# s-elkazdadi/ddp-pinocchio

Measured on AMD Instinct MI355X. Metric: DDP iterations/sec (fwd+bwd sweep), Talos nq=38 T=200, higher is better.
Workload: dtype f64

## Files before the change

ddp_pinocchio_amd/csrc/bwd.hip:

```cpp
#include <stdio.h>
#include <stdlib.h>

#include "internal.h"

namespace {

struct BwdParams {
  Dims d;
  const int64_t* ne;
  const int64_t* Epre;
  const double *lfx, *lfxx, *lx, *lu, *lxx, *lux, *luu, *fx, *fu, *fxx, *fux, *fuu;
  const double *eq_val, *eq_x, *eq_u, *eq_xx, *eq_ux, *eq_uu;
  const double *x, *mult_val, *mult_jac;
  double *fb_origin, *fb_val, *fb_jac, *vx_trace, *vxx_trace;
  double *ws_V, *ws_Q, *reg, *mu;
  int32_t* status;
  int64_t* restarts;
  const BwdJob* jobs;
  const BwdJob* jobs_half;
  int32_t njobs_half;
  int32_t half_mode;
  int32_t packed;
  const double *u, *ctrl_lo, *ctrl_hi;
  double* box_stat;
  int32_t has_tensors;
  int32_t sym_tensors;
};

constexpr int BS = 256;
typedef double f64x2 __attribute__((ext_vector_type(2)));

__global__ __launch_bounds__(BS) void bwd_init(BwdParams p) {
  const int b = blockIdx.x;
  const int s = p.status[b];
  if (s == 2) return;
  const int64_t n = p.d.n;
  double* Vx = p.ws_V + (int64_t)b * (n + n * n);
  double* Vxx = Vx + n;
  const double* lfx = p.lfx + (int64_t)b * n;
  const double* lfxx = p.lfxx + (int64_t)b * n * n;
  for (int64_t i = threadIdx.x; i < n; i += BS) Vx[i] = lfx[i];
  for (int64_t i = threadIdx.x; i < n * n; i += BS) Vxx[i] = lfxx[i];
  __syncthreads();
  if (threadIdx.x == 0 && s == 1) p.status[b] = 0;
}

template <int OC>
__device__ __forceinline__ void contract_slab(const double* __restrict__ Tn, int O_rt, int L, const double* s_v,
                                              double* s_part, double* out, int out_stride) {
  const int O = OC > 0 ? OC : O_rt;
  const int hp = O >> 1;
  const int ld = hp + 1;
  const int total = hp * L;
  const f64x2* __restrict__ T2 = reinterpret_cast<const f64x2*>(Tn);
  const int tid = threadIdx.x;
#pragma unroll 4
  for (int f = tid; f < total; f += BS) {
    const f64x2 a = __builtin_nontemporal_load(&T2[f]);
    const int j = f / hp;
    const int ip = f - j * hp;
    s_part[j * ld + ip] = s_v[2 * ip] * a.x + s_v[2 * ip + 1] * a.y;
  }
  __syncthreads();
  for (int j = tid; j < L; j += BS) {
    double s = 0.0;
    const double* pj = s_part + j * ld;
    for (int k = 0; k < hp; ++k) s += pj[k];
    out[j * out_stride] += s;
  }
  __syncthreads();
}

template <int NC, int MC>
__global__ __launch_bounds__(BS) void bwd_assemble(BwdParams p, int64_t t) {
  const int b = blockIdx.y;
  if (p.status[b] != 0) return;
  const BwdJob job = p.jobs[blockIdx.x];
  const int n = NC > 0 ? NC : (int)p.d.n;
  const int m = MC > 0 ? MC : (int)p.d.m;
  const int64_t T = p.d.T;
  const int e = (int)p.ne[t];
  const int64_t Eo = p.Epre[t];
  const int64_t Etot = p.d.Etot;
  const double mu = p.mu[b];
  const int tid = threadIdx.x;
  const int kind = job.kind, c0 = job.c0, cn = job.cn;
  const int rows = kind == 0 ? n + m : m;

  const double* Vx = p.ws_V + (int64_t)b * (n + (int64_t)n * n);
  const double* Vxx = Vx + n;
  double* Q = p.ws_Q + (int64_t)b * (n + m + (int64_t)n * n + (int64_t)m * n + (int64_t)m * m);
  double* Qx = Q;
  double* Qu = Qx + n;
  double* Qxx = Qu + m;
  double* Qux = Qxx + (int64_t)n * n;
  double* Quu = Qux + (int64_t)m * n;

  const int64_t bt = (int64_t)b * T + t;
  const double* fx = p.fx + bt * n * n;
  const double* fu = p.fu + bt * n * m;
  const double* eqv = p.eq_val + (int64_t)b * Etot + Eo;
  const double* eqx = p.eq_x + ((int64_t)b * Etot + Eo) * n;
  const double* equ = p.eq_u + ((int64_t)b * Etot + Eo) * m;
  const double* pe = p.mult_val + (int64_t)b * Etot + Eo;
  const double* pex = p.mult_jac + ((int64_t)b * Etot + Eo) * n;
// ... 333 lines not shown
      double s = r[i];
      for (int l = 0; l < i; ++l) s -= A[i + l * lda] * r[l];
      r[i] = s / A[i + i * lda];
    }
    for (int i = m - 1; i >= 0; --i) {
      double s = r[i];
      for (int l = i + 1; l < m; ++l) s -= A[l + i * lda] * r[l];
      r[i] = s / A[i + i * lda];
    }
  }
  __syncthreads();

  double* fbo = p.fb_origin + bt * nx;
  double* fbk = p.fb_val + bt * m;
  double* fbK = p.fb_jac + bt * m * n;
  const double* xt = p.x + ((int64_t)b * (T + 1) + t) * nx;
  for (int i = tid; i < nx; i += BS) fbo[i] = xt[i];
  for (int i = tid; i < m; i += BS) fbk[i] = R[i];
  for (int idx = tid; idx < m * n; idx += BS) fbK[idx] = R[idx % m + (idx / m + 1) * ldr];

  for (int i = tid; i < n; i += BS) {
    double s = 0.0;
    for (int l = 0; l < m; ++l) s += S[l + i * ldr] * R[l];
    const double v = Qx[i] + s;
    Vx[i] = v;
    if (p.vx_trace) p.vx_trace[bt * n + i] = v;
  }
  for (int idx = tid; idx < n * n; idx += BS) {
    const int i = idx % n, j = idx / n;
    double s = 0.0;
    const double* si = S + i * ldr;
    const double* kj = R + (j + 1) * ldr;
    for (int l = 0; l < m; ++l) s += si[l] * kj[l];
    const double v = Qxx[idx] + s;
    Vxx[idx] = v;
    if (p.vxx_trace) p.vxx_trace[bt * n * n + idx] = v;
  }
  if (t == 0 && tid == 0) p.status[b] = 2;
}

#include "bwd_fast.h"
#include "bwd_split.h"
#include "bwd_v2.h"

size_t assemble_lds_bytes(const ddp_hip_ctx* ctx, int cn_max) {
  const Dims& d = ctx->d;
  int64_t L = d.n > d.m ? d.n : d.m;
  int64_t words = d.n + d.emax + d.n * cn_max + (d.n + d.m) * cn_max + (d.n / 2 + 1) * L;
  return (size_t)words * sizeof(double);
}
size_t gains_lds_bytes(const ddp_hip_ctx* ctx) {
  const Dims& d = ctx->d;
  int64_t ld = d.m | 1;
  int64_t words = ld * d.m + ld * (d.n + 1) + ld * d.n;
  if (ctx->flags & DDP_HIP_FLAG_CONTROL_BOUNDS) words += ld * d.m + 9 * d.m;
  return (size_t)words * sizeof(double);
}

BwdParams make_params(ddp_hip_ctx* ctx, const SweepPlan& plan) {
  BwdParams p{};
  p.d = ctx->d;
  p.ne = ctx->ne_d;
  p.Epre = ctx->Epre_d;
  auto S = [&](int s) { return ctx->seq[s].ptr; };
  p.lfx = S(DDP_HIP_SEQ_LFX); p.lfxx = S(DDP_HIP_SEQ_LFXX);
  p.lx = S(DDP_HIP_SEQ_LX); p.lu = S(DDP_HIP_SEQ_LU); p.lxx = S(DDP_HIP_SEQ_LXX); p.lux = S(DDP_HIP_SEQ_LUX); p.luu = S(DDP_HIP_SEQ_LUU);
  p.fx = S(DDP_HIP_SEQ_FX); p.fu = S(DDP_HIP_SEQ_FU);
  p.fxx = S(DDP_HIP_SEQ_FXX); p.fux = S(DDP_HIP_SEQ_FUX); p.fuu = S(DDP_HIP_SEQ_FUU);
  p.eq_val = S(DDP_HIP_SEQ_EQ_VAL); p.eq_x = S(DDP_HIP_SEQ_EQ_X); p.eq_u = S(DDP_HIP_SEQ_EQ_U);
  p.eq_xx = S(DDP_HIP_SEQ_EQ_XX); p.eq_ux = S(DDP_HIP_SEQ_EQ_UX); p.eq_uu = S(DDP_HIP_SEQ_EQ_UU);
  p.x = S(DDP_HIP_SEQ_X);
  p.u = S(DDP_HIP_SEQ_U); p.ctrl_lo = S(DDP_HIP_SEQ_CTRL_LO); p.ctrl_hi = S(DDP_HIP_SEQ_CTRL_HI); p.box_stat = S(DDP_HIP_SEQ_BOX_STAT);
  p.mult_val = S(DDP_HIP_SEQ_MULT_VAL); p.mult_jac = S(DDP_HIP_SEQ_MULT_JAC);
  p.fb_origin = S(DDP_HIP_SEQ_FB_ORIGIN); p.fb_val = S(DDP_HIP_SEQ_FB_VAL); p.fb_jac = S(DDP_HIP_SEQ_FB_JAC);
  p.vx_trace = S(DDP_HIP_SEQ_VX_TRACE); p.vxx_trace = S(DDP_HIP_SEQ_VXX_TRACE);
  p.ws_V = ctx->ws_V; p.ws_Q = ctx->ws_Q; p.reg = ctx->reg_d; p.mu = ctx->mu_d;
  p.status = ctx->status_d; p.restarts = ctx->restarts_d;
  p.sym_tensors = plan.sym ? 1 : 0;
  p.jobs = plan.sym ? ctx->jobs_sym_d : ctx->jobs_d;
  p.jobs_half = plan.half_mode ? ctx->jobs_half_d : nullptr;
  p.njobs_half = plan.half_mode ? ctx->njobs_half : 0;
  p.half_mode = plan.half_mode;
  p.packed = plan.packed ? 1 : 0;
  p.has_tensors = (ctx->flags & DDP_HIP_FLAG_NO_TENSORS) ? 0 : 1;
  return p;
}

template <int NC, int MC, bool BOX = false>
int launch_sweep(ddp_hip_ctx* ctx, const BwdParams& p, size_t lds_a, size_t lds_g) {
  const Dims& d = ctx->d;
  hipLaunchKernelGGL(bwd_init, dim3((unsigned)d.batch), dim3(BS), 0, ctx->stream, p);
  for (int64_t t = d.T - 1; t >= 0; --t) {
    prof_begin(ctx, DDP_HIP_K_BWD_ASSEMBLE);
    hipLaunchKernelGGL((bwd_assemble<NC, MC>), dim3((unsigned)ctx->njobs, (unsigned)d.batch), dim3(BS), lds_a, ctx->stream, p, t);
    prof_end(ctx, DDP_HIP_K_BWD_ASSEMBLE);
    prof_begin(ctx, DDP_HIP_K_BWD_GAINS);
    hipLaunchKernelGGL((bwd_gains<NC, MC, BOX>), dim3((unsigned)d.batch), dim3(BS), lds_g, ctx->stream, p, t);
    prof_end(ctx, DDP_HIP_K_BWD_GAINS);
  }
  HIP_TRY(hipGetLastError());
  return DDP_HIP_OK;
}

template <int NC, int MC, bool BOX>
int enqueue_sweep_v2(ddp_hip_ctx* ctx, const BwdParams& p) {
  const Dims& d = ctx->d;
  const int cn_max = ctx->cbx > ctx->cbu ? ctx->cbx : ctx->cbu;
  const size_t lds_c = sizeof(double) * (size_t)(NC + (NC + MC) * cn_max + 2 * (NC / 2 + 1) * MC);
  const size_t lds_h = sizeof(double) * (size_t)(NC + 3 * NC + 2 * (MC / 2 + 1) * NC);
  const size_t lds_5 = sizeof(double) * (size_t)(NC * NC + NC * (NC + MC) + NC + d.emax);
  const unsigned nblk5 = (unsigned)((NC + MC + CB5 - 1) / CB5);
  const unsigned B = (unsigned)d.batch;
  hipLaunchKernelGGL(bwd_init, dim3(B), dim3(BS), 0, ctx->stream, p);
  for (int64_t t = d.T - 1; t >= 0; --t) {
    prof_begin(ctx, DDP_HIP_K_BWD_GAINS);
    hipLaunchKernelGGL((bwd_dense2<NC, MC>), dim3(nblk5, B), dim3(BS5), lds_5, ctx->stream, p, t);
    prof_end(ctx, DDP_HIP_K_BWD_GAINS);
    if (p.has_tensors) {
      prof_begin(ctx, DDP_HIP_K_BWD_ASSEMBLE);
      if (p.jobs_half && p.packed) hipLaunchKernelGGL((bwd_contract_half<NC, MC, true>), dim3((unsigned)p.njobs_half, B), dim3(BSF), lds_h, ctx->stream, p, t);
      else if (p.jobs_half) hipLaunchKernelGGL((bwd_contract_half<NC, MC, false>), dim3((unsigned)p.njobs_half, B), dim3(BSF), lds_h, ctx->stream, p, t);
      else hipLaunchKernelGGL((bwd_contract<NC, MC>), dim3((unsigned)ctx->njobs, B), dim3(BSF), lds_c, ctx->stream, p, t);
      prof_end(ctx, DDP_HIP_K_BWD_ASSEMBLE);
    }
    prof_begin(ctx, DDP_HIP_K_BWD_GAINS);
    hipLaunchKernelGGL((bwd_gains2<NC, MC, BOX>), dim3(B), dim3(BS4), 0, ctx->stream, p, t);
    prof_end(ctx, DDP_HIP_K_BWD_GAINS);
  }
  HIP_TRY(hipGetLastError());
  return DDP_HIP_OK;
}

template <int NC, int MC, bool BOX>
int build_sweep_graph(ddp_hip_ctx* ctx, const BwdParams& p0, uint64_t key_misc, ddp_hip_ctx::BwdGraph** out) {
  ddp_hip_ctx::BwdGraph* slot = &ctx->bwd_graph[ctx->bwd_graph_next];
  ctx->bwd_graph_next = (ctx->bwd_graph_next + 1) % 4;
  if (slot->exec) { (void)hipGraphExecDestroy(slot->exec); slot->exec = nullptr; }
  if (slot->graph) { (void)hipGraphDestroy(slot->graph); slot->graph = nullptr; }
  HIP_TRY(hipStreamBeginCapture(ctx->stream, hipStreamCaptureModeThreadLocal));
  const int rc = enqueue_sweep_v2<NC, MC, BOX>(ctx, p0);
  hipGraph_t graph = nullptr;
  const hipError_t e = hipStreamEndCapture(ctx->stream, &graph);
  if (rc != DDP_HIP_OK || e != hipSuccess || !graph) { (void)hipGetLastError(); if (graph) (void)hipGraphDestroy(graph); return rc != DDP_HIP_OK ? rc : DDP_HIP_E_HIP; }
  hipGraphExec_t exec = nullptr;
  if (hipGraphInstantiate(&exec, graph, nullptr, nullptr, 0) != hipSuccess) { (void)hipGetLastError(); (void)hipGraphDestroy(graph); return DDP_HIP_E_HIP; }
  slot->graph = graph; slot->exec = exec; slot->key_x = p0.x; slot->key_misc = key_misc;
  *out = slot;
  return DDP_HIP_OK;
}

template <int NC, int MC, bool BOX = false>
int launch_sweep_v2(ddp_hip_ctx* ctx, const BwdParams& p0) {
  const uint32_t bwd_mask = (2u << DDP_HIP_K_BWD_ASSEMBLE) | (2u << DDP_HIP_K_BWD_GAINS);
  if (ctx->sw.bwd_no_graph || (ctx->profile_mask & bwd_mask)) return enqueue_sweep_v2<NC, MC, BOX>(ctx, p0);
  const uint64_t key_misc = (uint64_t)p0.has_tensors | ((uint64_t)(p0.vx_trace != nullptr) << 1) | ((uint64_t)p0.sym_tensors << 2) | ((uint64_t)(p0.jobs_half != nullptr) << 3) | ((uint64_t)p0.half_mode << 4) | ((uint64_t)p0.packed << 8);
  auto find = [&](const void* key_x) -> ddp_hip_ctx::BwdGraph* {
    for (auto& g : ctx->bwd_graph)
      if (g.exec && g.key_x == key_x && g.key_misc == key_misc) return &g;
    return nullptr;
  };
  ddp_hip_ctx::BwdGraph* slot = find(p0.x);
  if (!slot) {
    int rc = build_sweep_graph<NC, MC, BOX>(ctx, p0, key_misc, &slot);
    if (rc != DDP_HIP_OK) return rc;
    const double* other = ctx->seq[DDP_HIP_SEQ_X_NEW].ptr;
    if (other && other != p0.x && !find(other)) {
      BwdParams p1 = p0;
      p1.x = other;
      p1.u = ctx->seq[DDP_HIP_SEQ_U_NEW].ptr;
      ddp_hip_ctx::BwdGraph* twin = nullptr;
      rc = build_sweep_graph<NC, MC, BOX>(ctx, p1, key_misc, &twin);
      if (rc != DDP_HIP_OK) return rc;
      slot = find(p0.x);
      if (!slot) return DDP_HIP_E_HIP;
    }
  }
  HIP_TRY(hipGraphLaunch(slot->exec, ctx->stream));
  return DDP_HIP_OK;
}

}

SweepPlan sweep_plan(const ddp_hip_ctx* ctx) {
  const Dims& d = ctx->d;
  const DevSwitches& sw = ctx->sw;
  SweepPlan s{};
  s.fast = d.n == 76 && d.m == 38 && d.emax <= 52 && !sw.generic_bwd;
  s.sym_ok = s.fast && ctx->jobs_sym_d && !sw.k3_no_sym;
  const TensorOrigin o = ctx->tensors.origin;
  s.sym = s.sym_ok && (o == TensorOrigin::Symmetric || o == TensorOrigin::Stencil);
  const bool half_ok = s.fast && ctx->jobs_half_d && !sw.k3_no_half;
  if (half_ok && s.sym && o == TensorOrigin::Stencil) { s.half_mode = 1; s.packed = ctx->tensors.packed; }
  else if (half_ok && o == TensorOrigin::Analytic1) s.half_mode = 2;
  return s;
}

int bwd_setup(ddp_hip_ctx* ctx) {
  const Dims& d = ctx->d;
  const int64_t n = d.n, m = d.m, B = d.batch;
  HIP_TRY(hipMalloc(&ctx->ws_V, sizeof(double) * (size_t)(B * (n + n * n))));
  HIP_TRY(hipMalloc(&ctx->ws_Q, sizeof(double) * (size_t)(B * (n + m + n * n + m * n + m * m))));
  HIP_TRY(hipMalloc(&ctx->reg_d, sizeof(double) * (size_t)B));
  HIP_TRY(hipMalloc(&ctx->mu_d, sizeof(double) * (size_t)B));
  HIP_TRY(hipMalloc(&ctx->status_d, sizeof(int32_t) * (size_t)B));
  HIP_TRY(hipMalloc(&ctx->restarts_d, sizeof(int64_t) * (size_t)B));

  int64_t units = 3 * n + m;
  int64_t want = 2048 / B;
  if (want < 1) want = 1;
  if (want > n + m) want = n + m;
  int64_t upj = (units + want - 1) / want;
  int64_t cbx = upj / 3; if (cbx < 1) cbx = 1; if (cbx > 8) cbx = 8;
  int64_t cbu = upj;     if (cbu < 1) cbu = 1; if (cbu > 16) cbu = 16;
  if (n == 76 && m == 38) { cbx = 1; cbu = 3; }
  if (ctx->sw.bwd_cbx) cbx = ctx->sw.bwd_cbx;
  if (ctx->sw.bwd_cbu) cbu = ctx->sw.bwd_cbu;
  ctx->cbx = (int32_t)cbx; ctx->cbu = (int32_t)cbu;
  std::vector<BwdJob> jobs;
  for (int64_t c = 0; c < n; c += cbx) jobs.push_back(BwdJob{0, (int32_t)c, (int32_t)((n - c) < cbx ? (n - c) : cbx), 0});
  for (int64_t c = 0; c < m; c += cbu) jobs.push_back(BwdJob{1, (int32_t)c, (int32_t)((m - c) < cbu ? (m - c) : cbu), 0});
  ctx->njobs = (int32_t)jobs.size();
  if (n == 76 && m == 38) {
    const size_t lds_5 = sizeof(double) * (size_t)(76 * 76 + 76 * (76 + 38) + 76 + d.emax);
    HIP_TRY(hipFuncSetAttribute(reinterpret_cast<const void*>(&bwd_dense2<76, 38>), hipFuncAttributeMaxDynamicSharedMemorySize, (int)lds_5));
  }
  if ((ctx->flags & DDP_HIP_FLAG_CONTROL_BOUNDS) && gains_lds_bytes(ctx) <= 160 * 1024) {
    HIP_TRY(hipFuncSetAttribute(reinterpret_cast<const void*>(&bwd_gains<0, 0, true>), hipFuncAttributeMaxDynamicSharedMemorySize, (int)gains_lds_bytes(ctx)));
  }
  {
    const size_t lds_a = assemble_lds_bytes(ctx, (int)(cbx > cbu ? cbx : cbu)), lds_g = gains_lds_bytes(ctx);
    if (lds_a > 64 * 1024 && lds_a <= 160 * 1024)
      HIP_TRY(hipFuncSetAttribute(reinterpret_cast<const void*>(&bwd_assemble<0, 0>), hipFuncAttributeMaxDynamicSharedMemorySize, (int)lds_a));
    if (!(ctx->flags & DDP_HIP_FLAG_CONTROL_BOUNDS) && lds_g > 64 * 1024 && lds_g <= 160 * 1024)
      HIP_TRY(hipFuncSetAttribute(reinterpret_cast<const void*>(&bwd_gains<0, 0, false>), hipFuncAttributeMaxDynamicSharedMemorySize, (int)lds_g));
  }
  HIP_TRY(hipMalloc(&ctx->jobs_d, sizeof(BwdJob) * jobs.size()));
  HIP_TRY(hipMemcpy(ctx->jobs_d, jobs.data(), sizeof(BwdJob) * jobs.size(), hipMemcpyHostToDevice));
  if (n == 76 && m == 38 && cbx == 1) {
    std::vector<BwdJob> js = jobs;
    for (auto& j : js) if (j.kind == 0 && j.c0 >= m) j.kind = 2;
    HIP_TRY(hipMalloc(&ctx->jobs_sym_d, sizeof(BwdJob) * js.size()));
    HIP_TRY(hipMemcpy(ctx->jobs_sym_d, js.data(), sizeof(BwdJob) * js.size(), hipMemcpyHostToDevice));
    std::vector<BwdJob> jh;
    for (int64_t c = 0; c < n; c += 2) jh.push_back(BwdJob{10, (int32_t)c, 2, 0});
    for (int64_t c = 0; c < m; c += 6) jh.push_back(BwdJob{11, (int32_t)c, (int32_t)((m - c) < 6 ? (m - c) : 6), 0});
    ctx->njobs_half = (int32_t)jh.size();
    HIP_TRY(hipMalloc(&ctx->jobs_half_d, sizeof(BwdJob) * jh.size()));
    HIP_TRY(hipMemcpy(ctx->jobs_half_d, jh.data(), sizeof(BwdJob) * jh.size(), hipMemcpyHostToDevice));
  }
  return DDP_HIP_OK;
}

void bwd_teardown(ddp_hip_ctx* ctx) {
  for (auto& g : ctx->bwd_graph) {
    if (g.exec) (void)hipGraphExecDestroy(g.exec);
    if (g.graph) (void)hipGraphDestroy(g.graph);
  }
  if (ctx->ws_V) (void)hipFree(ctx->ws_V);
  if (ctx->ws_Q) (void)hipFree(ctx->ws_Q);
  if (ctx->reg_d) (void)hipFree(ctx->reg_d);
  if (ctx->mu_d) (void)hipFree(ctx->mu_d);
  if (ctx->status_d) (void)hipFree(ctx->status_d);
  if (ctx->restarts_d) (void)hipFree(ctx->restarts_d);
  if (ctx->jobs_d) (void)hipFree(ctx->jobs_d);
  if (ctx->jobs_sym_d) (void)hipFree(ctx->jobs_sym_d);
  if (ctx->jobs_half_d) (void)hipFree(ctx->jobs_half_d);
}

int bwd_lds_check(const ddp_hip_ctx* ctx) {
  if (sweep_plan(ctx).fast) return DDP_HIP_OK;
  const int cn_max = ctx->cbx > ctx->cbu ? ctx->cbx : ctx->cbu;
  if (assemble_lds_bytes(ctx, cn_max) > 160 * 1024 || gains_lds_bytes(ctx) > 160 * 1024) return DDP_HIP_E_UNSUPPORTED;
  return DDP_HIP_OK;
}

extern "C" int ddp_hip_backward(ddp_hip_ctx* ctx, double* reg_io, double* mu_io, int64_t* restarts_out, int64_t max_restarts) {
  if (!ctx || !reg_io || !mu_io) return DDP_HIP_E_ARG;
  { const int rc_ = bwd_lds_check(ctx); if (rc_ != DDP_HIP_OK) return rc_; }
  const Dims& d = ctx->d;
  const int64_t B = d.batch;
  HIP_TRY(hipSetDevice(ctx->device));
  SweepPlan plan = sweep_plan(ctx);
  if (ctx->tensors.packed && !plan.packed) {
    const int rc_ = lin_materialize_fxx(ctx);
    if (rc_ != DDP_HIP_OK) return rc_;
    plan = sweep_plan(ctx);
  }
  BwdParams p = make_params(ctx, plan);
  if (p.has_tensors && (!p.fxx || !p.fux || !p.fuu)) return DDP_HIP_E_UNSUPPORTED;
  const bool box = (ctx->flags & DDP_HIP_FLAG_CONTROL_BOUNDS) != 0;
  if (box) { const int rc_ = box_check(ctx); if (rc_ != DDP_HIP_OK) return rc_; }
  if (p.has_tensors && ctx->tensors.mirror_pending && !plan.sym) { const int rc_ = lin_materialize_fxx(ctx); if (rc_ != DDP_HIP_OK) return rc_; }

  HIP_TRY(hipMemcpyAsync(ctx->reg_d, reg_io, sizeof(double) * (size_t)B, hipMemcpyHostToDevice, ctx->stream));
  HIP_TRY(hipMemcpyAsync(ctx->mu_d, mu_io, sizeof(double) * (size_t)B, hipMemcpyHostToDevice, ctx->stream));
  std::vector<int32_t> status((size_t)B);
  for (int64_t b = 0; b < B; ++b) status[(size_t)b] = ctx->active_h[(size_t)b] ? 0 : 2;
  HIP_TRY(hipMemcpyAsync(ctx->status_d, status.data(), sizeof(int32_t) * (size_t)B, hipMemcpyHostToDevice, ctx->stream));
  HIP_TRY(hipMemsetAsync(ctx->restarts_d, 0, sizeof(int64_t) * (size_t)B, ctx->stream));

  const int cn_max = ctx->cbx > ctx->cbu ? ctx->cbx : ctx->cbu;
  const size_t lds_a = assemble_lds_bytes(ctx, cn_max);
  const size_t lds_g = gains_lds_bytes(ctx);

  bool any_restart = false;
  int rc = DDP_HIP_OK;
  for (int64_t attempt = 0;; ++attempt) {
    if (plan.fast) rc = box ? launch_sweep_v2<76, 38, true>(ctx, p) : launch_sweep_v2<76, 38>(ctx, p);
    else if (d.n == 12 && d.m == 6) rc = box ? launch_sweep<12, 6, true>(ctx, p, lds_a, lds_g) : launch_sweep<12, 6>(ctx, p, lds_a, lds_g);
    else rc = box ? launch_sweep<0, 0, true>(ctx, p, lds_a, lds_g) : launch_sweep<0, 0>(ctx, p, lds_a, lds_g);
    if (rc != DDP_HIP_OK) return rc;
    HIP_TRY(hipMemcpyAsync(status.data(), ctx->status_d, sizeof(int32_t) * (size_t)B, hipMemcpyDeviceToHost, ctx->stream));
    HIP_TRY(hipStreamSynchronize(ctx->stream));
    bool failed = false;
    for (int64_t b = 0; b < B; ++b) failed |= status[(size_t)b] == 1;
    if (!failed) break;
    any_restart = true;
    if (max_restarts >= 0 && attempt >= max_restarts) { rc = DDP_HIP_E_MAX_RESTARTS; break; }
  }
  HIP_TRY(hipMemcpyAsync(reg_io, ctx->reg_d, sizeof(double) * (size_t)B, hipMemcpyDeviceToHost, ctx->stream));
  HIP_TRY(hipMemcpyAsync(mu_io, ctx->mu_d, sizeof(double) * (size_t)B, hipMemcpyDeviceToHost, ctx->stream));
  if (restarts_out)
    HIP_TRY(hipMemcpyAsync(restarts_out, ctx->restarts_d, sizeof(int64_t) * (size_t)B, hipMemcpyDeviceToHost, ctx->stream));
  HIP_TRY(hipStreamSynchronize(ctx->stream));
  if (rc != DDP_HIP_OK) return rc;
  return any_restart ? DDP_HIP_EV_LLT_RESTART : DDP_HIP_OK;
}

#ifdef BWD_STAMPS
extern "C" int ddp_hip_debug_stamps(unsigned long long* out32) {
  return hipMemcpyFromSymbol(out32, HIP_SYMBOL(g_bwd_stamps), sizeof(unsigned long long) * 32) == hipSuccess ? 0 : -2;
}
#endif
```

ddp_pinocchio_amd/csrc/bwd_split.h:

```cpp
#pragma once

template <int N, int M>
__global__ __launch_bounds__(BSF, BWD_WAVES_PER_SIMD) void bwd_contract(BwdParams p, int64_t t) {
  int b, jb;
  {
    const int njobs = (int)gridDim.x, B = (int)gridDim.y;
    const int lin = blockIdx.y * njobs + blockIdx.x;
    if ((B & 7) == 0) {
      const int xcd = lin & 7, k = lin >> 3;
      b = xcd + 8 * (k / njobs);
      jb = k % njobs;
    } else { b = blockIdx.y; jb = blockIdx.x; }
  }
  if (p.status[b] != 0) return;
  const BwdJob job = p.jobs[jb];
  constexpr int n = N, m = M;
  const int64_t T = p.d.T;
  const int tid = threadIdx.x;
  const int kind = job.kind, c0 = job.c0, cn = job.cn;
  const int rows = kind == 1 ? m : n + m;
  static_assert(N == 2 * M, "half-slabs: the state tangent is twice the control dimension");
  const int64_t bt = (int64_t)b * T + t;

  const double* Vx = p.ws_V + (int64_t)b * (n + n * n);
// ... 161 lines not shown
          top[0] = tw.x;
          if (xcol && (j % M) != (slab % M)) top[1] = tw.y;
        } else {
          const double* colp = unit_base(u) + (int64_t)tid * n;
          top[0] = colp[slab % M];
          if (xcol && (j % M) != (slab % M)) top[1] = colp[j % M];
        }
      }
    }
  };
  if (U > 0) issue(0, buf0, top0);
  if (U > 1) issue(1, buf1, top1);
  if (U > 2) issue(2, buf2, top2);
  double* dst = nullptr;
  double* dm = nullptr;
  double old_d = 0.0, old_m = 0.0;
  static_assert(3 * N <= BSF, "one output entry per lane");
  if (tid < U * N) {
    const int u = tid / N, jj = tid - u * N;
    int slab, j; bool xcol;
    if (col_info(u, jj, slab, j, xcol)) {
      if (kind == 10) {
        if (u < 2) { dst = Cxx + j + slab * n; if (j > slab && !m1) dm = Cxx + slab + j * n; }
        else dst = Cux + j + slab * m;
      } else { dst = Cuu + j + slab * m; if (j > slab && !m1) dm = Cuu + slab + j * m; }
      old_d = *dst;
      if (dm) old_m = *dm;
    }
  }
  for (int i = tid; i < n; i += BSF) s_v[i] = Vx[i];
  __syncthreads();
  auto step = [&](int u, f64x2 (&buf)[HS::R], double (&top)[2]) {
    double* sp = (u & 1) ? s_p1 : s_p0;
#pragma unroll
    for (int r = 0; r < HS::R; ++r) {
      const int f = tid + r * BSF;
      if (r < HS::R - 1 || f < HS::TOTAL) {
        const int jj = f / HS::HP, ip = f - jj * HS::HP;
        const f64x2 vv = *reinterpret_cast<const f64x2*>(s_v + M + 2 * ip);
        sp[jj * HS::LD + ip] = vv.x * buf[r].x + vv.y * buf[r].y;
      }
    }
    __syncthreads();
    if (tid < n) {
      int slab, j; bool xcol;
      const bool need = col_info(u, tid, slab, j, xcol);
      double sacc = 0.0;
      if (need && kind == 10 && !m1) {
        const int ra = slab % M, rb = xcol ? j % M : ra;
        const int lo = ra < rb ? ra : rb, hi = ra < rb ? rb : ra;
        const double tlo = ra <= rb ? top[0] : top[1], thi = ra <= rb ? (ra == rb ? 0.0 : top[1]) : top[0];
        if (lo == hi) {
          const int e = lo & ~1;
          const f64x2 vv = *reinterpret_cast<const f64x2*>(s_v + e);
          const double tx = (lo & 1) ? 0.0 : tlo, ty = (lo & 1) ? tlo : 0.0;
          sacc += vv.x * tx + vv.y * ty;
        } else if ((lo >> 1) == (hi >> 1)) {
          const f64x2 vv = *reinterpret_cast<const f64x2*>(s_v + lo);
          sacc += vv.x * tlo + vv.y * thi;
        } else {
          const f64x2 va = *reinterpret_cast<const f64x2*>(s_v + (lo & ~1));
          const f64x2 vb = *reinterpret_cast<const f64x2*>(s_v + (hi & ~1));
          sacc += va.x * ((lo & 1) ? 0.0 : tlo) + va.y * ((lo & 1) ? tlo : 0.0);
          sacc += vb.x * ((hi & 1) ? 0.0 : thi) + vb.y * ((hi & 1) ? thi : 0.0);
        }
      }
      const double* pj = sp + tid * HS::LD;
#pragma unroll
      for (int k = 0; k < HS::HP; ++k) sacc += pj[k];
      s_out[u * N + tid] = sacc;
    }
  };
  if (U > 0) step(0, buf0, top0);
  if (U > 1) step(1, buf1, top1);
  if (U > 2) step(2, buf2, top2);
  (void)buf3; (void)top3;
  __syncthreads();
  if (dst) {
    const double v = s_out[tid];
    *dst = old_d + v;
    if (dm) *dm = old_m + v;
  }
}
```

ddp_pinocchio_amd/csrc/internal.h:

```cpp
#pragma once

#include <hip/hip_runtime.h>
#include <stdint.h>

#include <vector>

#include "cost_block.h"
#include "ddp_hip/ddp_hip.h"

#define DDP_MAXJ DDP_HIP_MAX_JOINTS

struct DevModel {
  int32_t kind, nv;
  int32_t ff, nj, nq, pad0_;
  double mass, length;
  double gravity[3];
  double dt, c;
  int32_t parent[DDP_MAXJ];
  int32_t jtype[DDP_MAXJ];
  double axis[DDP_MAXJ][3];
  double Rp[DDP_MAXJ][9];
  double pp[DDP_MAXJ][3];
  double I6[DDP_MAXJ][21];
  int32_t has_child[DDP_MAXJ];
  int32_t first_contrib[DDP_MAXJ];
  int32_t last_child[DDP_MAXJ];
  int32_t slot_up[DDP_MAXJ];
  int32_t slot_down[DDP_MAXJ];
  int32_t n_slots;
  int32_t n_levels, max_level_width;
  int32_t lvl_start[DDP_MAXJ + 1];
  int32_t lvl_joint[DDP_MAXJ];
  int32_t child_start[DDP_MAXJ + 1];
  int32_t child_list[DDP_MAXJ];
  int32_t eq_kind, eq_advance, frame_joint, first_order_fd, fd_mode, pad_;
  double frame_off[3];
};

struct Dims {
  int64_t T, n, m, nx, nv, batch;
  int64_t Etot;
  int64_t emax;
};

struct SeqBuf {
  double* ptr = nullptr;
  int64_t size = 0;
};

struct BwdJob {
  int32_t kind;
  int32_t c0, cn;
  int32_t pad_;
};

struct DevSwitches {
  bool generic_bwd = false;
  bool k3_no_sym = false;
  bool k3_no_half = false;
  bool k3_no_pack = false;
  bool fxx_full = false;
  bool no_static = false;
  bool no_qcache = false;
  bool qcache_dense = false;
  bool cfg_full_aba = false;
  bool ana_own_aba = false;
  bool ana_split = false;
  bool ana_eq_kernel = false;
  bool bwd_no_graph = false;
  bool solve_sync = false;
  bool fwd_no_pipe = false;
  bool lin_serial = false;
  int32_t lin_forks = 0;
  int32_t bwd_cbx = 0, bwd_cbu = 0;
  int64_t qws_bt = 0;
  int64_t ana_bt = 0;
};

struct SweepPlan {
  bool fast;
  bool sym_ok;
  bool sym;
  int32_t half_mode;
  bool packed;
};

enum class LinFirst : int32_t {
  Base,
  AnalyticSmall,
  AnalyticWave,
  AnalyticFF,
  FdStatic,
  FdGeneric,
};
enum class LinSecond : int32_t {
  None,
  Zeros,
  Mode2Static,
  Mode2Caches,
  Mode2Plain,
  Mode1Small,
  Mode1Wave,
};
enum class LinEq : int32_t {
  None,
  PerLane,
  Analytic,
  Chain,
};
enum LinFork : uint32_t {
  LIN_FORK_CFG = 1,
  LIN_FORK_SPINE = 2,
  LIN_FORK_DEFAULT = LIN_FORK_CFG | LIN_FORK_SPINE,
};
enum class LinEqJac : int32_t { None, Fd, FfLookahead };
enum class LinEqSecond : int32_t { None, Zeros, Mode2, Mode1Small, Mode1Wave };
struct LinPlan {
  int32_t refuse = 0;
  int32_t nj = 0;
  int32_t topo = 0;
  LinFirst first = LinFirst::Base;
  LinSecond second = LinSecond::None;
  LinEq eq = LinEq::None;
  LinEqJac eq_jac = LinEqJac::None;
  LinEqSecond eq_second = LinEqSecond::None;
  bool eq_inline = false;
  bool accel_static = false;
  bool accel_with_u = false;
  bool m1_fused = false;
  int32_t ncfg = 0, nvcfg = 0;
  bool qc_sparse = false;
  bool has_tensors = false;
  bool skip_top = false;
  bool skip_qv_mirror = false;
  bool pack = false;
  bool ws_lin = false, ws_qws = false, ws_qws2 = false;
  bool ws_ana_T = false, ws_ana_M = false, ws_ana_M0 = false, ws_ana_A = false, ws_ana_F = false;
  bool ws_eq = false;
  bool ana_sliced = false;
  int64_t eq_fxk_off = 0, eq_c_off = 0, eq_words = 0;
  uint32_t forks = 0;
  int32_t lin_path = 0, first_order = 0;
};
DevSwitches read_switches();
LinPlan lin_plan_decide(const DevModel& m, const Dims& d, uint32_t flags, const DevSwitches& sw, int topo_id, bool sweep_sym_ok);

enum class TensorOrigin : int32_t {
  Unknown,
  Symmetric,
  Stencil,
  Analytic1,
};
struct TensorState {
  TensorOrigin origin = TensorOrigin::Unknown;
  bool mirror_pending = false;
  bool packed = false;
};

struct LinCall {
  bool ana_A_fresh = false;
  bool ana_M0_fresh = false;
  bool fuu_zero = false;
};

struct ProfSlot {
  std::vector<hipEvent_t> starts, stops;
  size_t used = 0;
  double total_ms = 0;
  int64_t launches = 0;
};

struct ddp_hip_ctx {
  int device = 0;
  int cu_count = 0;
  uint32_t flags = 0;
  hipStream_t stream = nullptr;
  Dims d{};
  std::vector<int64_t> ne_h, Epre_h;
  int64_t* ne_d = nullptr;
  int64_t* Epre_d = nullptr;
  double* target_d = nullptr;
  DevModel model_h{};
  DevModel* model_d = nullptr;
  SeqBuf seq[DDP_HIP_SEQ_COUNT];
  DevSwitches sw;

  double* ws_V = nullptr;
  double* ws_Q = nullptr;
  double* reg_d = nullptr;
  double* mu_d = nullptr;
  int32_t* status_d = nullptr;
  int64_t* restarts_d = nullptr;
  BwdJob* jobs_d = nullptr;
  BwdJob* jobs_half_d = nullptr;
  int32_t njobs_half = 0;
  TensorState tensors;
  BwdJob* jobs_sym_d = nullptr;
  int32_t njobs = 0;
  int32_t cbx = 0, cbu = 0;
  struct BwdGraph { const void* key_x = nullptr; uint64_t key_misc = 0; hipGraphExec_t exec = nullptr; hipGraph_t graph = nullptr; };
  BwdGraph bwd_graph[4];
  int bwd_graph_next = 0;

  double* fw_x = nullptr;
  double* fw_u = nullptr;
  double* fw_dcost = nullptr;
  double* fw_cost = nullptr;
  double* fw_cost_old = nullptr;
  double* step_d = nullptr;
  int32_t* fw_state_d = nullptr;
  double* fw_dcost_acc_d = nullptr;
  int32_t n_alpha_max = 8;
  double* pick_pair_d = nullptr;

  double* eq_ws = nullptr;
  double* lin_ws = nullptr;
  LinPlan plan;
  double* lin_qws = nullptr;
  int64_t lin_qws_bt = 0;
  double* lin_qws2 = nullptr;
  hipStream_t lin_stream2 = nullptr;
  hipEvent_t lin_ev_up[2] = {nullptr, nullptr}, lin_ev_dn[2] = {nullptr, nullptr};
  hipEvent_t lin_ev_fork = nullptr, lin_ev_done = nullptr, lin_ev_rows = nullptr;
  bool lin_side_busy = false;
  double* ana_T = nullptr;
  double* ana_M = nullptr;
  double* ana_F = nullptr;
  double* ana_M0 = nullptr;
  double* ana_A = nullptr;
  int64_t ana_nbt = 0;

  std::vector<int32_t> active_h;
  bool all_active = true;

  CostBlock cost[COST_COUNT];
  int32_t fc_nf = 0;
  int32_t fc_joint[DDP_HIP_MAX_COST_FRAMES] = {};
  double fc_off[DDP_HIP_MAX_COST_FRAMES][3] = {};
  int32_t ob_np = 0, ob_no = 0;
  int32_t ob_joint[DDP_HIP_MAX_COLLISION_POINTS] = {};
  double ob_off[DDP_HIP_MAX_COLLISION_POINTS][3] = {};
  double ob_radius[DDP_HIP_MAX_COLLISION_POINTS] = {};
  int32_t ob_kind[DDP_HIP_MAX_OBSTACLES] = {};
  double* ob_clear_d = nullptr;
  int32_t sc_np = 0, sc_npair = 0;
  int32_t sc_joint[DDP_HIP_MAX_COLLISION_POINTS] = {};
  double sc_off[DDP_HIP_MAX_COLLISION_POINTS][3] = {};
  double sc_radius[DDP_HIP_MAX_COLLISION_POINTS] = {};
  int32_t sc_pa[DDP_HIP_MAX_COLLISION_PAIRS] = {}, sc_pb[DDP_HIP_MAX_COLLISION_PAIRS] = {};
  double* sc_clear_d = nullptr;
  int32_t rf_np = 0;
  int32_t rf_ja[DDP_HIP_MAX_FRAME_PAIRS] = {}, rf_jb[DDP_HIP_MAX_FRAME_PAIRS] = {};
  double rf_offa[DDP_HIP_MAX_FRAME_PAIRS][3] = {}, rf_offb[DDP_HIP_MAX_FRAME_PAIRS][3] = {};
  double* rf_err_d = nullptr;

  bool box_dirty = false;

  bool async_mode = false;
  uint32_t profile_mask = 0;
  ProfSlot prof[DDP_HIP_K_COUNT];
};

#define HIP_TRY(expr)                                   \
  do {                                                  \
    hipError_t e__ = (expr);                            \
    if (e__ != hipSuccess) { (void)hipGetLastError(); return DDP_HIP_E_HIP; } \
  } while (0)

#define END_SYNC(ctx) do { if (!(ctx)->async_mode) HIP_TRY(hipStreamSynchronize((ctx)->stream)); } while (0)

inline hipError_t lin_fork(ddp_hip_ctx* ctx) {
  hipError_t e = hipEventRecord(ctx->lin_ev_fork, ctx->stream);
  if (e == hipSuccess) e = hipStreamWaitEvent(ctx->lin_stream2, ctx->lin_ev_fork, 0);
  if (e == hipSuccess) ctx->lin_side_busy = true;
  return e;
}
inline hipError_t lin_join(ddp_hip_ctx* ctx) {
  if (!ctx->lin_side_busy) return hipSuccess;
// ... 35 lines not shown
```

ddp_pinocchio_amd/csrc/lin_plan.cpp:

```cpp
#include <stdlib.h>

#include "internal.h"

DevSwitches read_switches() {
  auto on = [](const char* name) { return getenv(name) != nullptr; };
  auto knob = [](const char* name, int lo, int hi) { const char* ev = getenv(name); const int v = ev ? atoi(ev) : 0; return v >= lo && v <= hi ? v : 0; };
  DevSwitches sw;
  sw.generic_bwd = on("DDP_HIP_GENERIC_BWD");
  sw.k3_no_sym = on("DDP_HIP_K3_NO_SYM");
  sw.k3_no_half = on("DDP_HIP_K3_NO_HALF");
  sw.k3_no_pack = on("DDP_HIP_K3_NO_PACK");
  sw.fxx_full = on("DDP_HIP_FXX_FULL");
  sw.no_static = on("DDP_HIP_NO_STATIC");
  sw.no_qcache = on("DDP_HIP_NO_QCACHE");
  sw.qcache_dense = on("DDP_HIP_QCACHE_DENSE");
  sw.cfg_full_aba = on("DDP_HIP_CFG_FULL_ABA");
  sw.ana_own_aba = on("DDP_HIP_ANA_OWN_ABA");
  sw.ana_split = on("DDP_HIP_ANA_SPLIT");
  sw.ana_eq_kernel = on("DDP_HIP_ANA_EQ_KERNEL");
  sw.bwd_no_graph = on("DDP_HIP_BWD_NO_GRAPH");
  sw.solve_sync = on("DDP_HIP_SOLVE_SYNC");
  sw.fwd_no_pipe = on("DDP_HIP_FWD_NO_PIPE");
  sw.lin_serial = on("DDP_HIP_LIN_SERIAL");
  sw.lin_forks = knob("DDP_HIP_LIN_FORKS", 1, 3);
  sw.bwd_cbx = knob("DDP_HIP_BWD_CBX", 1, 8);
  sw.bwd_cbu = knob("DDP_HIP_BWD_CBU", 1, 16);
  sw.qws_bt = knob("DDP_HIP_QWS_BT", 16, 65536);
  sw.ana_bt = knob("DDP_HIP_ANA_BT", 1, 65536);
  return sw;
}

LinPlan lin_plan_decide(const DevModel& m, const Dims& d, uint32_t flags, const DevSwitches& sw, int topo_id, bool sweep_sym_ok) {
  LinPlan pl;
  const bool tree = m.kind == DDP_HIP_MODEL_TREE, ff = m.ff != 0, fo_fd = m.first_order_fd != 0;
  const bool tensors = !(flags & DDP_HIP_FLAG_NO_TENSORS);
  const bool analytic = tree && !fo_fd;
  const int mode = m.fd_mode;
  const int64_t nv = d.nv, K = m.eq_advance;
  pl.has_tensors = tensors;
  pl.nj = nv <= 1 ? 1 : (nv <= 6 && !ff) ? 6 : nv <= 38 ? 38 : 64;
  const bool small = pl.nj <= 6;
  const bool wave = analytic && !small && !ff;

  if (mode == 1 && fo_fd && tensors) pl.refuse = DDP_HIP_E_UNSUPPORTED;
  if (analytic && ff && nv > 38) pl.refuse = DDP_HIP_E_UNSUPPORTED;
  if (wave && m.max_level_width > 64) pl.refuse = DDP_HIP_E_UNSUPPORTED;
  if (wave && d.Etot > 0 && (K < 1 || K > 2)) pl.refuse = DDP_HIP_E_UNSUPPORTED;

  const int topo = (tree && !ff && !sw.no_static) ? topo_id : 0;
  const bool stencil_caches = tree && mode == 2 && tensors && !ff && !sw.no_qcache;
  const bool accel = topo && wave && mode == 1 && tensors && !sw.ana_own_aba;
  if (stencil_caches) { pl.ncfg = (int32_t)nv + 1; pl.nvcfg = 2 * (int32_t)nv + 1; }
  else if ((topo && fo_fd) || accel) { pl.ncfg = 1; pl.nvcfg = 1; }
  pl.ws_lin = pl.ncfg > 0;
  pl.topo = pl.ws_lin ? topo : 0;
  pl.ws_qws = pl.topo != 0;

  if (analytic) pl.first = small ? LinFirst::AnalyticSmall : ff ? LinFirst::AnalyticFF : LinFirst::AnalyticWave;
  else if (fo_fd) pl.first = pl.topo ? LinFirst::FdStatic : LinFirst::FdGeneric;
  else pl.first = LinFirst::Base;

  if (!tensors) pl.second = LinSecond::None;
  else if (mode == 0) pl.second = LinSecond::Zeros;
  else if (mode == 1) pl.second = small ? LinSecond::Mode1Small : LinSecond::Mode1Wave;
  else if (pl.ncfg > 1) pl.second = pl.topo ? LinSecond::Mode2Static : LinSecond::Mode2Caches;
  else pl.second = LinSecond::Mode2Plain;
  pl.ws_qws2 = pl.second == LinSecond::Mode2Static && sw.cfg_full_aba;
  pl.qc_sparse = pl.second == LinSecond::Mode2Static && !sw.qcache_dense && !sw.cfg_full_aba;
  pl.skip_top = pl.topo && mode == 2 && tensors && !sw.fxx_full;
  pl.skip_qv_mirror = pl.skip_top && sweep_sym_ok;
  pl.pack = pl.skip_qv_mirror && pl.second == LinSecond::Mode2Static && !sw.k3_no_half && !sw.k3_no_pack;

  const bool m1_wave = wave && pl.second == LinSecond::Mode1Wave;
  pl.ana_sliced = analytic && !small;
  pl.ws_ana_T = wave && sw.ana_split;
  pl.ws_ana_M = wave && (sw.ana_split || (m1_wave && d.Etot > 0));
  pl.ws_ana_M0 = m1_wave && !sw.ana_split;
  pl.ws_ana_A = pl.accel_static = accel;
  pl.accel_with_u = accel && d.Etot > 0;
  pl.ws_ana_F = m1_wave && d.Etot > 0;

  pl.ws_eq = d.Etot > 0 && tree && (fo_fd || ff);
  if (d.Etot > 0) {
    pl.eq = (small && !pl.ws_eq) ? LinEq::PerLane : wave ? LinEq::Analytic : LinEq::Chain;
    if (pl.eq == LinEq::Chain && K > 1) pl.eq_jac = fo_fd ? LinEqJac::Fd : LinEqJac::FfLookahead;
    pl.eq_second = !tensors ? LinEqSecond::None : mode == 0 ? LinEqSecond::Zeros : mode == 2 ? LinEqSecond::Mode2
                   : small ? LinEqSecond::Mode1Small : LinEqSecond::Mode1Wave;
    pl.m1_fused = m1_wave;
    pl.eq_inline = m1_wave && !sw.ana_split && m.eq_kind == DDP_HIP_EQ_CONFIG && !sw.ana_eq_kernel;
  }
  if (pl.ws_eq) {
    pl.eq_fxk_off = d.batch * d.T * K * d.nx;
    pl.eq_c_off = pl.eq_fxk_off + d.batch * d.T * (K > 1 ? K - 1 : 0) * d.n * d.n;
    pl.eq_words = pl.eq_c_off + d.batch * d.T * d.emax * d.n;
// ... 60 lines not shown
```

Baseline: 791.6.

## Pack second-order tensor contraction into balanced multi-unit jobs for half-mode backward

Adds a new backward tensor-contraction kernel that takes precomputed work units, each a list of up to four column runs across fxx/fux/fuu slabs. Triangular column tails are paired (c with n-c) so every unit carries a similar amount of work, and several units are grouped per block to cut the block count and balance load. The old column-job path is kept behind an environment switch. The cost is more complex indexing and extra LDS use per block.

```diff
diff --git a/ddp_pinocchio_amd/csrc/bwd.hip b/ddp_pinocchio_amd/csrc/bwd.hip
--- a/ddp_pinocchio_amd/csrc/bwd.hip
+++ b/ddp_pinocchio_amd/csrc/bwd.hip
@@ -21,6 +21,8 @@
   int32_t njobs_half;
   int32_t half_mode;
   int32_t packed;
+  const K3hUnit* units_half;
+  int32_t njobs_units;
   const double *u, *ctrl_lo, *ctrl_hi;
   double* box_stat;
   int32_t has_tensors;
@@ -520,6 +522,9 @@
   p.njobs_half = plan.half_mode ? ctx->njobs_half : 0;
   p.half_mode = plan.half_mode;
   p.packed = plan.packed ? 1 : 0;
+  const bool full_units = plan.half_mode == 1 && plan.packed && !ctx->sw.k3h_column_jobs;
+  p.units_half = full_units ? ctx->units_half_d : nullptr;
+  p.njobs_units = full_units ? ctx->njobs_units : 0;
   p.has_tensors = (ctx->flags & DDP_HIP_FLAG_NO_TENSORS) ? 0 : 1;
   return p;
 }
@@ -546,6 +551,7 @@
   const int cn_max = ctx->cbx > ctx->cbu ? ctx->cbx : ctx->cbu;
   const size_t lds_c = sizeof(double) * (size_t)(NC + (NC + MC) * cn_max + 2 * (NC / 2 + 1) * MC);
   const size_t lds_h = sizeof(double) * (size_t)(NC + 3 * NC + 2 * (MC / 2 + 1) * NC);
+  const size_t lds_u = sizeof(double) * (size_t)(NC + K3H_UNITS_PER_JOB * NC + 2 * (MC / 2 + 1) * NC + 4 * NC);
   const size_t lds_5 = sizeof(double) * (size_t)(NC * NC + NC * (NC + MC) + NC + d.emax);
   const unsigned nblk5 = (unsigned)((NC + MC + CB5 - 1) / CB5);
   const unsigned B = (unsigned)d.batch;
@@ -556,7 +562,8 @@
     prof_end(ctx, DDP_HIP_K_BWD_GAINS);
     if (p.has_tensors) {
       prof_begin(ctx, DDP_HIP_K_BWD_ASSEMBLE);
-      if (p.jobs_half && p.packed) hipLaunchKernelGGL((bwd_contract_half<NC, MC, true>), dim3((unsigned)p.njobs_half, B), dim3(BSF), lds_h, ctx->stream, p, t);
+      if (p.units_half) hipLaunchKernelGGL((bwd_contract_units<NC, MC, K3H_UNITS_PER_JOB>), dim3((unsigned)p.njobs_units, B), dim3(BSF), lds_u, ctx->stream, p, t);
+      else if (p.jobs_half && p.packed) hipLaunchKernelGGL((bwd_contract_half<NC, MC, true>), dim3((unsigned)p.njobs_half, B), dim3(BSF), lds_h, ctx->stream, p, t);
       else if (p.jobs_half) hipLaunchKernelGGL((bwd_contract_half<NC, MC, false>), dim3((unsigned)p.njobs_half, B), dim3(BSF), lds_h, ctx->stream, p, t);
       else hipLaunchKernelGGL((bwd_contract<NC, MC>), dim3((unsigned)ctx->njobs, B), dim3(BSF), lds_c, ctx->stream, p, t);
       prof_end(ctx, DDP_HIP_K_BWD_ASSEMBLE);
@@ -591,7 +598,7 @@
 int launch_sweep_v2(ddp_hip_ctx* ctx, const BwdParams& p0) {
   const uint32_t bwd_mask = (2u << DDP_HIP_K_BWD_ASSEMBLE) | (2u << DDP_HIP_K_BWD_GAINS);
   if (ctx->sw.bwd_no_graph || (ctx->profile_mask & bwd_mask)) return enqueue_sweep_v2<NC, MC, BOX>(ctx, p0);
-  const uint64_t key_misc = (uint64_t)p0.has_tensors | ((uint64_t)(p0.vx_trace != nullptr) << 1) | ((uint64_t)p0.sym_tensors << 2) | ((uint64_t)(p0.jobs_half != nullptr) << 3) | ((uint64_t)p0.half_mode << 4) | ((uint64_t)p0.packed << 8);
+  const uint64_t key_misc = (uint64_t)p0.has_tensors | ((uint64_t)(p0.vx_trace != nullptr) << 1) | ((uint64_t)p0.sym_tensors << 2) | ((uint64_t)(p0.jobs_half != nullptr) << 3) | ((uint64_t)p0.half_mode << 4) | ((uint64_t)p0.packed << 8) | ((uint64_t)(p0.units_half != nullptr) << 9);
   auto find = [&](const void* key_x) -> ddp_hip_ctx::BwdGraph* {
     for (auto& g : ctx->bwd_graph)
       if (g.exec && g.key_x == key_x && g.key_misc == key_misc) return &g;
@@ -679,12 +686,15 @@
     for (auto& j : js) if (j.kind == 0 && j.c0 >= m) j.kind = 2;
     HIP_TRY(hipMalloc(&ctx->jobs_sym_d, sizeof(BwdJob) * js.size()));
     HIP_TRY(hipMemcpy(ctx->jobs_sym_d, js.data(), sizeof(BwdJob) * js.size(), hipMemcpyHostToDevice));
-    std::vector<BwdJob> jh;
-    for (int64_t c = 0; c < n; c += 2) jh.push_back(BwdJob{10, (int32_t)c, 2, 0});
-    for (int64_t c = 0; c < m; c += 6) jh.push_back(BwdJob{11, (int32_t)c, (int32_t)((m - c) < 6 ? (m - c) : 6), 0});
+    const std::vector<BwdJob> jh = k3h_column_jobs((int)n, (int)m);
     ctx->njobs_half = (int32_t)jh.size();
     HIP_TRY(hipMalloc(&ctx->jobs_half_d, sizeof(BwdJob) * jh.size()));
     HIP_TRY(hipMemcpy(ctx->jobs_half_d, jh.data(), sizeof(BwdJob) * jh.size(), hipMemcpyHostToDevice));
+    std::vector<K3hUnit> us = k3h_full_units((int)n, (int)m);
+    if (!k3h_units_in_bounds(us, (int)n, (int)m)) return DDP_HIP_E_ARG;
+    ctx->njobs_units = k3h_pad_to_jobs(us, K3H_UNITS_PER_JOB);
+    HIP_TRY(hipMalloc(&ctx->units_half_d, sizeof(K3hUnit) * us.size()));
+    HIP_TRY(hipMemcpy(ctx->units_half_d, us.data(), sizeof(K3hUnit) * us.size(), hipMemcpyHostToDevice));
   }
   return DDP_HIP_OK;
 }
@@ -703,6 +713,7 @@
   if (ctx->jobs_d) (void)hipFree(ctx->jobs_d);
   if (ctx->jobs_sym_d) (void)hipFree(ctx->jobs_sym_d);
   if (ctx->jobs_half_d) (void)hipFree(ctx->jobs_half_d);
+  if (ctx->units_half_d) (void)hipFree(ctx->units_half_d);
 }
 
 int bwd_lds_check(const ddp_hip_ctx* ctx) {
diff --git a/ddp_pinocchio_amd/csrc/bwd_jobs.h b/ddp_pinocchio_amd/csrc/bwd_jobs.h
--- /dev/null
+++ b/ddp_pinocchio_amd/csrc/bwd_jobs.h
@@ -0,0 +1,97 @@
+#pragma once
+
+#include <stdint.h>
+
+#include <vector>
+
+#ifdef __HIPCC__
+#define K3H_HD __host__ __device__ inline
+#else
+#define K3H_HD inline
+#endif
+
+struct BwdJob {
+  int32_t kind;
+  int32_t c0, cn;
+  int32_t pad_;
+};
+
+#ifndef K3H_UNITS_PER_JOB
+#define K3H_UNITS_PER_JOB 3
+#endif
+constexpr int K3H_RUNS = 4;
+enum : int16_t { K3H_FXX = 0, K3H_FUX = 1, K3H_FUU = 2 };
+
+struct K3hRun {
+  int16_t tensor, slab, j0, cnt;
+};
+struct K3hUnit {
+  K3hRun run[K3H_RUNS];
+};
+
+struct K3hCol {
+  int tensor, slab, j;
+  bool need;
+};
+K3H_HD K3hCol k3h_col(const K3hUnit& un, int jj) {
+  const int s1 = un.run[0].cnt, s2 = s1 + un.run[1].cnt, s3 = s2 + un.run[2].cnt, s4 = s3 + un.run[3].cnt;
+  const int k = (jj >= s1) + (jj >= s2) + (jj >= s3);
+  const K3hRun r = k == 0 ? un.run[0] : k == 1 ? un.run[1] : k == 2 ? un.run[2] : un.run[3];
+  const int s = k == 0 ? 0 : k == 1 ? s1 : k == 2 ? s2 : s3;
+  return K3hCol{r.tensor, r.slab, r.j0 + (jj - s), jj < s4};
+}
+K3H_HD int k3h_unit_columns(const K3hUnit& un) { return un.run[0].cnt + un.run[1].cnt + un.run[2].cnt + un.run[3].cnt; }
+
+inline std::vector<BwdJob> k3h_column_jobs(int n, int m) {
+  std::vector<BwdJob> jh;
+  for (int c = 0; c < n; c += 2) jh.push_back(BwdJob{10, c, 2, 0});
+  for (int c = 0; c < m; c += 6) jh.push_back(BwdJob{11, c, (m - c) < 6 ? (m - c) : 6, 0});
+  return jh;
+}
+inline std::vector<K3hUnit> k3h_column_job_units(const BwdJob& job, int n, int m) {
+  std::vector<K3hUnit> us;
+  auto tail = [](int16_t tensor, int c, int len) { return K3hRun{tensor, (int16_t)c, (int16_t)c, (int16_t)(len - c)}; };
+  const int c0 = job.c0;
+  if (job.kind == 10) {
+    us.push_back(K3hUnit{{tail(K3H_FXX, c0, n), {}, {}, {}}});
+    us.push_back(K3hUnit{{tail(K3H_FXX, c0 + 1, n), {}, {}, {}}});
+    us.push_back(K3hUnit{{K3hRun{K3H_FUX, (int16_t)c0, 0, (int16_t)m}, K3hRun{K3H_FUX, (int16_t)(c0 + 1), 0, (int16_t)m}, {}, {}}});
+  } else {
+    for (int u = 0; u < job.cn / 2; ++u) us.push_back(K3hUnit{{tail(K3H_FUU, c0 + 2 * u, m), tail(K3H_FUU, c0 + 2 * u + 1, m), {}, {}}});
+  }
+  return us;
+}
+
+inline std::vector<K3hUnit> k3h_full_units(int n, int m) {
+  std::vector<K3hUnit> us;
+  auto tail = [](int16_t tensor, int c, int len) { return K3hRun{tensor, (int16_t)c, (int16_t)c, (int16_t)(len - c)}; };
+  us.push_back(K3hUnit{{tail(K3H_FXX, 0, n), {}, {}, {}}});
+  for (int c = 1; c < m; ++c) us.push_back(K3hUnit{{tail(K3H_FXX, c, n), tail(K3H_FXX, n - c, n), {}, {}}});
+  us.push_back(K3hUnit{{tail(K3H_FXX, m, n), {}, {}, {}}});
+  for (int c = 0; c < n; c += 2) us.push_back(K3hUnit{{K3hRun{K3H_FUX, (int16_t)c, 0, (int16_t)m}, K3hRun{K3H_FUX, (int16_t)(c + 1), 0, (int16_t)m}, {}, {}}});
+  for (int c = 1; c < m / 2; c += 2) {
+    K3hUnit un{{tail(K3H_FUU, c, m), tail(K3H_FUU, m - c, m), {}, {}}};
+    if (c + 1 < m / 2) { un.run[2] = tail(K3H_FUU, c + 1, m); un.run[3] = tail(K3H_FUU, m - c - 1, m); }
+    us.push_back(un);
+  }
+  us.push_back(K3hUnit{{tail(K3H_FUU, 0, m), tail(K3H_FUU, m / 2, m), {}, {}}});
+  return us;
+}
+
+inline bool k3h_units_in_bounds(const std::vector<K3hUnit>& us, int n, int m) {
+  for (const K3hUnit& un : us) {
+    if (k3h_unit_columns(un) > n) return false;
+    for (const K3hRun& r : un.run) {
+      if (r.cnt < 0 || r.j0 < 0 || r.slab < 0 || r.tensor < K3H_FXX || r.tensor > K3H_FUU) return false;
+      if (r.cnt == 0) { if (r.tensor || r.slab || r.j0) return false; continue; }
+      const int slabs = r.tensor == K3H_FUU ? m : n, cols = r.tensor == K3H_FXX ? n : m;
+      if (r.slab >= slabs || r.j0 + r.cnt > cols) return false;
+    }
+  }
+  return true;
+}
+
+inline int k3h_pad_to_jobs(std::vector<K3hUnit>& us, int units_per_job) {
+  while (us.size() % (size_t)units_per_job) us.push_back(K3hUnit{});
+  return (int)(us.size() / (size_t)units_per_job);
+}
diff --git a/ddp_pinocchio_amd/csrc/bwd_split.h b/ddp_pinocchio_amd/csrc/bwd_split.h
--- a/ddp_pinocchio_amd/csrc/bwd_split.h
+++ b/ddp_pinocchio_amd/csrc/bwd_split.h
@@ -267,3 +267,138 @@
     if (dm) *dm = old_m + v;
   }
 }
+
+template <int N, int M, int UPJ>
+__global__ __launch_bounds__(BSF, BWD_WAVES_PER_SIMD) void bwd_contract_units(BwdParams p, int64_t t) {
+  int b, jb;
+  {
+    const int njobs = (int)gridDim.x, B = (int)gridDim.y;
+    const int lin = blockIdx.y * njobs + blockIdx.x;
+    if ((B & 7) == 0) {
+      const int xcd = lin & 7, k = lin >> 3;
+      b = xcd + 8 * (k / njobs);
+      jb = k % njobs;
+    } else { b = blockIdx.y; jb = blockIdx.x; }
+  }
+  if (p.status[b] != 0) return;
+  constexpr int n = N, m = M;
+  static_assert(N == 2 * M && M % 2 == 0, "lower halves of M rows, in row pairs");
+  using HS = HalfShape<N, M>;
+  constexpr int W = HS::HP + 1;
+  constexpr int R = (W * N + BSF - 1) / BSF;
+  static_assert(UPJ * N <= BSF, "one output entry per lane");
+  const K3hUnit* units = p.units_half + (int64_t)jb * UPJ;
+  const int64_t T = p.d.T;
+  const int tid = threadIdx.x;
+  const int64_t bt = (int64_t)b * T + t;
+  const double* Vx = p.ws_V + (int64_t)b * (n + n * n);
+  double* C = p.ws_Q + (int64_t)b * (n + m + n * n + m * n + m * m) + n + m;
+  constexpr int OXX = 0, OUX = n * n, OUU = n * n + m * n;
+  extern __shared__ __attribute__((aligned(16))) double smem[];
+  double* s_v = smem;
+  double* s_out = s_v + n;
+  double* s_p0 = s_out + UPJ * N;
+  double* s_p1 = s_p0 + HS::LD * N;
+  f64x2* s_t0 = reinterpret_cast<f64x2*>(s_p1 + HS::LD * N);
+  f64x2* s_t1 = s_t0 + N;
+  auto run_base = [&](const K3hRun& r) -> const f64x2* {
+    const double* slab = r.tensor == K3H_FXX ? p.fxx + (bt * n + r.slab) * (int64_t)(n * n)
+                       : r.tensor == K3H_FUX ? p.fux + (bt * n + r.slab) * (int64_t)(n * m)
+                                             : p.fuu + (bt * m + r.slab) * (int64_t)(n * m);
+    return reinterpret_cast<const f64x2*>(slab + (int64_t)r.j0 * (M + 2));
+  };
+  f64x2 buf[UPJ][R];
+#pragma unroll
+  for (int u = 0; u < UPJ; ++u) {
+    const K3hUnit un = units[u];
+    const int e1 = W * un.run[0].cnt, e2 = e1 + W * un.run[1].cnt, e3 = e2 + W * un.run[2].cnt, e4 = e3 + W * un.run[3].cnt;
+    const f64x2 *b0 = run_base(un.run[0]), *b1 = run_base(un.run[1]) - e1, *b2 = run_base(un.run[2]) - e2, *b3 = run_base(un.run[3]) - e3;
+#pragma unroll
+    for (int r = 0; r < R; ++r) {
+      const int f = tid + r * BSF;
+      const int k = (f >= e1) + (f >= e2) + (f >= e3);
+      const f64x2* src = (k == 0 ? b0 : k == 1 ? b1 : k == 2 ? b2 : b3) + f;
+      const int tensor = k == 0 ? un.run[0].tensor : k == 1 ? un.run[1].tensor : k == 2 ? un.run[2].tensor : un.run[3].tensor;
+      const bool need = f < e4 && !(tensor == K3H_FUU && f % W == 0);
+      if (need) buf[u][r] = BWD_NT ? __builtin_nontemporal_load(src) : *src;
+      else buf[u][r] = f64x2{0.0, 0.0};
+    }
+  }
+  int dst = -1, dm = -1;
+  double old_d = 0.0, old_m = 0.0;
+  if (tid < UPJ * N) {
+    const int u = tid / N, jj = tid - u * N;
+    const K3hCol c = k3h_col(units[u], jj);
+    if (c.need) {
+      if (c.tensor == K3H_FUX) dst = OUX + c.j + c.slab * m;
+      else {
+        const int o = c.tensor == K3H_FXX ? OXX : OUU, ld = c.tensor == K3H_FXX ? n : m;
+        dst = o + c.j + c.slab * ld;
+        if (c.j > c.slab) dm = o + c.slab + c.j * ld;
+      }
+      old_d = C[dst];
+      if (dm >= 0) old_m = C[dm];
+    }
+  }
+  for (int i = tid; i < n; i += BSF) s_v[i] = Vx[i];
+  __syncthreads();
+#pragma unroll
+  for (int u = 0; u < UPJ; ++u) {
+    double* sp = (u & 1) ? s_p1 : s_p0;
+    f64x2* st = (u & 1) ? s_t1 : s_t0;
+#pragma unroll
+    for (int r = 0; r < R; ++r) {
+      const int f = tid + r * BSF;
+      if (r < R - 1 || f < W * N) {
+        const int jj = f / W, w = f - jj * W;
+        if (w == 0) st[jj] = buf[u][r];
+        else {
+          const int ip = w - 1;
+          const f64x2 vv = *reinterpret_cast<const f64x2*>(s_v + M + 2 * ip);
+          sp[jj * HS::LD + ip] = vv.x * buf[u][r].x + vv.y * buf[u][r].y;
+        }
+      }
+    }
+    __syncthreads();
+    if (tid < n) {
+      const K3hCol c = k3h_col(units[u], tid);
+      const int slab = c.slab, j = c.j;
+      const bool xcol = c.tensor == K3H_FXX;
+      double sacc = 0.0;
+      if (c.need && c.tensor != K3H_FUU) {
+        const f64x2 tw = st[tid];
+        double top[2];
+        top[0] = tw.x;
+        top[1] = 0.0;
+        if (xcol && (j % M) != (slab % M)) top[1] = tw.y;
+        const int ra = slab % M, rb = xcol ? j % M : ra;
+        const int lo = ra < rb ? ra : rb, hi = ra < rb ? rb : ra;
+        const double tlo = ra <= rb ? top[0] : top[1], thi = ra <= rb ? (ra == rb ? 0.0 : top[1]) : top[0];
+        if (lo == hi) {
+          const int e = lo & ~1;
+          const f64x2 vv = *reinterpret_cast<const f64x2*>(s_v + e);
+          const double tx = (lo & 1) ? 0.0 : tlo, ty = (lo & 1) ? tlo : 0.0;
+          sacc += vv.x * tx + vv.y * ty;
+        } else if ((lo >> 1) == (hi >> 1)) {
+          const f64x2 vv = *reinterpret_cast<const f64x2*>(s_v + lo);
+          sacc += vv.x * tlo + vv.y * thi;
+        } else {
+          const f64x2 va = *reinterpret_cast<const f64x2*>(s_v + (lo & ~1));
+          const f64x2 vb = *reinterpret_cast<const f64x2*>(s_v + (hi & ~1));
+          sacc += va.x * ((lo & 1) ? 0.0 : tlo) + va.y * ((lo & 1) ? tlo : 0.0);
+          sacc += vb.x * ((hi & 1) ? 0.0 : thi) + vb.y * ((hi & 1) ? thi : 0.0);
+        }
+      }
+      const double* pj = sp + tid * HS::LD;
+#pragma unroll
+      for (int k = 0; k < HS::HP; ++k) sacc += pj[k];
+      s_out[u * N + tid] = sacc;
+    }
+  }
+  __syncthreads();
+  if (dst >= 0) {
+    const double v = s_out[tid];
+    C[dst] = old_d + v;
+    if (dm >= 0) C[dm] = old_m + v;
+  }
+}
diff --git a/ddp_pinocchio_amd/csrc/internal.h b/ddp_pinocchio_amd/csrc/internal.h
--- a/ddp_pinocchio_amd/csrc/internal.h
+++ b/ddp_pinocchio_amd/csrc/internal.h
@@ -5,6 +5,7 @@
 
 #include <vector>
 
+#include "bwd_jobs.h"
 #include "cost_block.h"
 #include "ddp_hip/ddp_hip.h"
 
@@ -48,17 +49,12 @@
   int64_t size = 0;
 };
 
-struct BwdJob {
-  int32_t kind;
-  int32_t c0, cn;
-  int32_t pad_;
-};
-
 struct DevSwitches {
   bool generic_bwd = false;
   bool k3_no_sym = false;
   bool k3_no_half = false;
   bool k3_no_pack = false;
+  bool k3h_column_jobs = false;
   bool fxx_full = false;
   bool no_static = false;
   bool no_qcache = false;
@@ -194,6 +190,8 @@
   BwdJob* jobs_d = nullptr;
   BwdJob* jobs_half_d = nullptr;
   int32_t njobs_half = 0;
+  K3hUnit* units_half_d = nullptr;
+  int32_t njobs_units = 0;
   TensorState tensors;
   BwdJob* jobs_sym_d = nullptr;
   int32_t njobs = 0;
diff --git a/ddp_pinocchio_amd/csrc/lin_plan.cpp b/ddp_pinocchio_amd/csrc/lin_plan.cpp
--- a/ddp_pinocchio_amd/csrc/lin_plan.cpp
+++ b/ddp_pinocchio_amd/csrc/lin_plan.cpp
@@ -10,6 +10,7 @@
   sw.k3_no_sym = on("DDP_HIP_K3_NO_SYM");
   sw.k3_no_half = on("DDP_HIP_K3_NO_HALF");
   sw.k3_no_pack = on("DDP_HIP_K3_NO_PACK");
+  sw.k3h_column_jobs = on("DDP_HIP_K3H_COLUMN_JOBS");
   sw.fxx_full = on("DDP_HIP_FXX_FULL");
   sw.no_static = on("DDP_HIP_NO_STATIC");
   sw.no_qcache = on("DDP_HIP_NO_QCACHE");
```

Measured after the change: 807.0, median of 6. 1.9% higher.
